# gk969/stm32-speech-recognition

Hardware: AMD Instinct MI355X
Metric: utterances/sec (256-frame, 100 templates) (higher is better)
Workload: dtype int32

## Files before the change

### include/sr_engine.h

```cpp
#ifndef SR_ENGINE_H
#define SR_ENGINE_H

#include <stddef.h>
#include <stdint.h>

#ifdef __cplusplus
extern "C" {
#endif

#define SR_OK 0
#define SR_ERR_NO_DEVICE 1
#define SR_ERR_BAD_CONFIG 2
#define SR_ERR_BAD_ARG 3
#define SR_ERR_NO_TEMPLATES 4
#define SR_ERR_HIP 5

#define SR_ST_OK 0
#define SR_ST_VAD_FAIL 1
#define SR_ST_MFCC_FAIL 2
#define SR_ST_SEG_OOB 3

#define SR_DIS_ERR 0xFFFFFFFFu
#define SR_SAVE_MASK 12345u

// ... 32 lines not shown
    uint32_t frm_num;
    uint32_t status;
} sr_result;

typedef struct sr_engine sr_engine;

void sr_default_config(sr_config *cfg);
int sr_create(const sr_config *cfg, sr_engine **out);
void sr_destroy(sr_engine *h);
const char *sr_last_error(void);

typedef struct sr_tables {
    uint16_t *hamm;
    uint16_t *tri_cen;
    uint16_t *tri_even;
    uint16_t *tri_odd;
    int8_t *dct;
    int16_t *tw_kr;
    int16_t *tw_ki;
    uint32_t *log_thr;
} sr_tables;
int sr_build_tables(const sr_config *cfg, const sr_tables *out);
int sr_build_tie_table(int8_t *out);
int sr_log_table_mismatches(void);
uint32_t sr_mag_cheap_bound(const sr_engine *h);
uint32_t sr_mag_table(uint16_t *out, uint32_t n);

int sr_set_templates(sr_engine *h, const void *store, uint32_t n_slots, uint32_t stride_bytes);
int sr_set_templates_dense(sr_engine *h, const int16_t *mfcc, const uint32_t *frames, const uint8_t *valid,
                           uint32_t n_templates, uint32_t tpl_stride);
uint32_t sr_num_templates(const sr_engine *h);
int sr_train_store(sr_engine *h, const uint16_t *pcm, uint64_t pcm_stride, uint32_t buf_len, uint32_t n,
                   const uint32_t *slot, void *store, uint32_t n_slots, uint32_t stride_bytes, uint32_t *status);

int sr_recognize_batch(sr_engine *h, const uint16_t *pcm, uint64_t pcm_stride, uint32_t buf_len, uint32_t B,
                       sr_result *results, uint32_t *scores, int16_t *mfcc, sr_vad_rec *vad);
int sr_recognize_batch_dev(sr_engine *h, const uint16_t *d_pcm, uint64_t pcm_stride, uint32_t buf_len, uint32_t B,
                           sr_result *d_results, uint32_t *d_scores, int16_t *d_mfcc, sr_vad_rec *d_vad,
                           void *stream);
int sr_recognize_batch_packed12(sr_engine *h, const uint8_t *packed, uint64_t row_stride_bytes, uint32_t buf_len, uint32_t B,
                                sr_result *results, uint32_t *scores, int16_t *mfcc, sr_vad_rec *vad);

int sr_recognize_segments_batch(sr_engine *h, const uint16_t *pcm, uint64_t pcm_stride, uint32_t buf_len, uint32_t B,
                                sr_result *results, uint32_t *scores, sr_vad_rec *vad);
int sr_recognize_segments_batch_dev(sr_engine *h, const uint16_t *d_pcm, uint64_t pcm_stride, uint32_t buf_len,
                                    uint32_t B, sr_result *d_results, uint32_t *d_scores, sr_vad_rec *d_vad,
// ... 498 lines not shown
```

### stm32_speech_recognition_amd/csrc/k_mfcc.hip

```cpp
#include "sr_fft_dev.h"

#include <type_traits>

namespace sr {

constexpr int kMfccWaves = 4;
constexpr int kFramesPerWave = 16, kFramesPerWaveMid = 4, kFramesPerWaveSmall = 1;
#ifndef SR_MAG_TAB_BINS
#define SR_MAG_TAB_BINS 8
#endif
constexpr int mfcc_tab_bins(int fpw) { return fpw == kFramesPerWave ? SR_MAG_TAB_BINS : 0; }
static_assert(SR_MAG_TAB_BINS == 0 || SR_MAG_TAB_BINS == 4 || SR_MAG_TAB_BINS == 8, "table bins per lane");
#ifndef SR_MFCC_PIPE
#define SR_MFCC_PIPE 1
#endif
#ifndef SR_MFCC_PIPE_PEEL
#define SR_MFCC_PIPE_PEEL 1
#endif
#ifndef SR_MFCC_PIPE_VMCNT
#define SR_MFCC_PIPE_VMCNT (SR_MFCC_PIPE_PEEL ? 3 : 0)
#endif
static_assert(SR_MFCC_PIPE_VMCNT == 0 || (SR_MFCC_PIPE_VMCNT == 3 && SR_MFCC_PIPE_PEEL), "younger loads counted by the wait");
constexpr bool mfcc_pipelined(int fpw) { return SR_MFCC_PIPE && mfcc_tab_bins(fpw) == 8; }
#ifndef SR_MFCC_TM_REGS
#define SR_MFCC_TM_REGS 1
#endif
#ifdef SR_INJECT_LDS_RACE
#undef SR_MFCC_TM_REGS
#define SR_MFCC_TM_REGS 0
#endif
constexpr bool mfcc_tm_regs(int fpw) { return SR_MFCC_TM_REGS && mfcc_pipelined(fpw); }
constexpr int kMelPad = kMel + 1;
__device__ __forceinline__ constexpr int mel_prefix_word(int j) { return 64 * (j & 7) + (j >> 3); }
#pragma clang diagnostic push
#pragma clang diagnostic ignored "-Winline-asm"
__device__ __forceinline__ void mel_prefix_store(uint32_t base, const uint32_t (&pe)[8], const uint32_t (&po)[8])
{
    static_assert(kBins == 512, "the offsets below are written out for two halves of 512 words");
    asm volatile("s_mov_b32 m0, %16\n\ts_nop 0\n\t"
                 "ds_write_addtid_b32 %0\n\tds_write_addtid_b32 %1 offset:256\n\tds_write_addtid_b32 %2 offset:512\n\t"
                 "ds_write_addtid_b32 %3 offset:768\n\tds_write_addtid_b32 %4 offset:1024\n\tds_write_addtid_b32 %5 offset:1280\n\t"
                 "ds_write_addtid_b32 %6 offset:1536\n\tds_write_addtid_b32 %7 offset:1792\n\t"
                 "ds_write_addtid_b32 %8 offset:2048\n\tds_write_addtid_b32 %9 offset:2304\n\tds_write_addtid_b32 %10 offset:2560\n\t"
                 "ds_write_addtid_b32 %11 offset:2816\n\tds_write_addtid_b32 %12 offset:3072\n\tds_write_addtid_b32 %13 offset:3328\n\t"
                 "ds_write_addtid_b32 %14 offset:3584\n\tds_write_addtid_b32 %15 offset:3840"
                 :
                 : "v"(pe[0]), "v"(pe[1]), "v"(pe[2]), "v"(pe[3]), "v"(pe[4]), "v"(pe[5]), "v"(pe[6]), "v"(pe[7]), "v"(po[0]),
                   "v"(po[1]), "v"(po[2]), "v"(po[3]), "v"(po[4]), "v"(po[5]), "v"(po[6]), "v"(po[7]), "s"(base)
                 : "m0", "memory");
}
__device__ __forceinline__ void mel_energy_store(uint32_t base, const uint32_t (&en)[8])
{
    static_assert(4 * energy_plane(1) == 256 && 4 * energy_plane(2) == 528 && 4 * energy_plane(3) == 784 && 4 * energy_plane(4) == 1040 &&
                      4 * energy_plane(5) == 1296 && 4 * energy_plane(6) == 1568 && 4 * energy_plane(7) == 1824 && kBins == kEnergyBins,
                  "the offsets below are written out for these plane bases");
    asm volatile("s_mov_b32 m0, %8\n\ts_nop 0\n\t"
                 "ds_write_addtid_b32 %0\n\tds_write_addtid_b32 %1 offset:256\n\tds_write_addtid_b32 %2 offset:528\n\t"
                 "ds_write_addtid_b32 %3 offset:784\n\tds_write_addtid_b32 %4 offset:1040\n\tds_write_addtid_b32 %5 offset:1296\n\t"
                 "ds_write_addtid_b32 %6 offset:1568\n\tds_write_addtid_b32 %7 offset:1824"
                 :
                 : "v"(en[0]), "v"(en[2]), "v"(en[4]), "v"(en[6]), "v"(en[1]), "v"(en[3]), "v"(en[5]), "v"(en[7]), "s"(base)
                 : "m0", "memory");
}
#pragma clang diagnostic pop
constexpr int mfcc_wave_lds_words(int fpw) { return kXchgWords + fpw * kMelPad + 64; }

template <typename Base>
struct MfccTabArgs : Base {
    const uint16_t *mag_q;
    uint32_t mag_table_off;
};
template <typename Base>
constexpr int mfcc_feat_kind<MfccTabArgs<Base>> = mfcc_feat_kind<Base>;
template <typename Base>
static MfccTabArgs<Base> mfcc_tab_args(const Base &b, const MfccMagTab &tab)
{
    MfccTabArgs<Base> r;
    static_cast<Base &>(r) = b;
    r.mag_q = tab.mag_q;
    r.mag_table_off = tab.mag_table_off;
    return r;
}

template <int kFPW, typename Args = MfccTabArgs<MfccArgs>>
__global__ void __launch_bounds__(64 * kMfccWaves, 4) k_mfcc(const Args a)
{
    constexpr int kFeat = mfcc_feat_kind<Args>;
    constexpr uint32_t kFeatW = (kFeat == SR_FEAT_FFT || kFeat == SR_FEAT_MAG) ? kBins : kMel;
    constexpr int kWaveLdsWords = mfcc_wave_lds_words(kFPW);
    constexpr int kTabBins = mfcc_tab_bins(kFPW);
    constexpr bool kPipe = mfcc_pipelined(kFPW);
    constexpr bool kTmRegs = mfcc_tm_regs(kFPW);
    extern __shared__ __attribute__((aligned(16))) uint32_t smem[];
    __shared__ uint32_t s_dctM[kCoef * kMelPad];
    __shared__ int s_dctS[kCoef * kMelPad];
    __shared__ u32x4 s_tw3[kTw3Row * 4], s_tw5[8 * 64];
    __shared__ u32x4 s_tm[4 * 64];
    const int lane = threadIdx.x & 63, w = __builtin_amdgcn_readfirstlane(threadIdx.x >> 6);
    uint32_t *buf = smem + w * kWaveLdsWords;
    uint32_t *xw = buf;
    uint32_t *powb = buf + kXchgWords, *moff = powb + kFPW * kMelPad;
    const uint32_t buf_lds = (uint32_t)(uintptr_t)(const __attribute__((address_space(3))) uint32_t *)buf;
    (void)buf_lds;

    for (int i = threadIdx.x; i < kCoef * kMel; i += blockDim.x) {
        const int c = a.t.dct[i], o = (i / kMel) * kMelPad + i % kMel;
        s_dctM[o] = (uint32_t)(((c < 0 ? -c : c) * 262144 + 99) / 100);
        s_dctS[o] = (c > 0) - (c < 0);
    }
    __syncthreads();

    LaneTw tw;
    load_lane_tw(a.t, lane, lane >> 4, tw);
    real_leg_tw(tw);
    if (w == 0 && (lane & 15) == 0) {
        const uint32_t *f = &tw.s3[0][0][0];
        const int d0 = lane >> 4;
#pragma unroll
        for (int c = 0; c < 8; c++) s_tw3[d0 * kTw3Row + c] = u32x4{f[4 * c], f[4 * c + 1], f[4 * c + 2], f[4 * c + 3]};
    }
    if (w == 1 % kMfccWaves) store_tw32(s_tw5, lane, tw.s5);
    u32x4 tm_r[4];
    if constexpr (kTmRegs) {
#pragma unroll
        for (int c = 0; c < 2; c++) {
            tm_r[c] = *(const u32x4 *)(a.t.tri_even_m + 8 * lane + 4 * c);
            tm_r[c + 2] = *(const u32x4 *)(a.t.tri_odd_m + 8 * lane + 4 * c);
        }
    }
#ifndef SR_INJECT_LDS_RACE
    if (!kTmRegs && w == 2 % kMfccWaves) {
#pragma unroll
        for (int c = 0; c < 2; c++) {
            s_tm[64 * c + lane] = *(const u32x4 *)(a.t.tri_even_m + 8 * lane + 4 * c);
            s_tm[64 * (c + 2) + lane] = *(const u32x4 *)(a.t.tri_odd_m + 8 * lane + 4 * c);
        }
    }
#endif
    __syncthreads();
#ifdef SR_INJECT_LDS_RACE
    if (w == 2 % kMfccWaves) {
#if SR_INJECT_LDS_RACE >= 2
        __builtin_amdgcn_s_sleep(127);
#endif
#pragma unroll
        for (int c = 0; c < 2; c++) {
            s_tm[64 * c + lane] = *(const u32x4 *)(a.t.tri_even_m + 8 * lane + 4 * c);
            s_tm[64 * (c + 2) + lane] = *(const u32x4 *)(a.t.tri_odd_m + 8 * lane + 4 * c);
        }
    }
#endif
    int hamm_m[3];
#pragma unroll
    for (int k = 0; k < 3; k++) hamm_m[k] = (lane + 64 * k < kFrameLen) ? hamm_fused_multiplier(a.t.hamm[lane + 64 * k]) : 0;
    int f_lo = 0, p_hi = 0, p_lo = 0, x_hi = 0, x_lo = 0;
    if (lane < kMel) {
        const int h = lane;
        f_lo = (h == 0) ? 0 : (int)a.t.tri_cen[h - 1];
        const int f_hi = (h == kMel - 1) ? kBins : (int)a.t.tri_cen[h + 1];
        const int ih = f_hi - 1, il = f_lo ? f_lo - 1 : 0, half = (h & 1) ? kBins : 0;
        p_hi = half + mel_prefix_word(ih), x_hi = (ih >> 3) > 0 ? (ih >> 3) - 1 : 0;
        p_lo = half + mel_prefix_word(il), x_lo = (il >> 3) > 0 ? (il >> 3) - 1 : 0;
    }
    const uint64_t mag_p = (uint64_t)a.mag_q;
    const u32x4 mag_rs = {(uint32_t)mag_p, (uint32_t)(mag_p >> 32) | (2u << 16), kMagTabEntries, 0x00027000u};
    const uint32_t tw_off = 32u * (uint32_t)lane;
    const int c0 = energy_read_base(lane), c1 = c0 + 4;

    uint32_t item = blockIdx.x;
    uint32_t nx_nfrm = 0;
    int nx_mid = 0, nx_seg0 = 0;
    if (item < a.n_items) {
        const sr_vad_rec *rec = a.vad + item / a.tiles;
        nx_nfrm = rec->frm_num;
        nx_mid = (int)rec->atap.mid_val;
        nx_seg0 = rec->seg[0];
    }
    for (; item < a.n_items; item += gridDim.x) {
        const uint32_t b = item / a.tiles, tile = item - b * a.tiles;
        const uint32_t nfrm = nx_nfrm;
        const int mid = nx_mid, seg0 = nx_seg0;
        if (item + gridDim.x < a.n_items) {
            const sr_vad_rec *rec = a.vad + (item + gridDim.x) / a.tiles;
            nx_nfrm = rec->frm_num;
            nx_mid = (int)rec->atap.mid_val;
            nx_seg0 = rec->seg[0];
        }
        const uint16_t *row = a.pcm + (uint64_t)b * a.pcm_stride;
        int16_t *out = a.mfcc + (uint64_t)b * a.max_frames * kCoef;
        const uint32_t f0 = tile * (kMfccWaves * kFPW) + w * kFPW;
        uint32_t *frow = nullptr;
        if constexpr (kFeat != 0) frow = a.feat + (uint64_t)b * a.max_frames * kFeatW;
        uint32_t nf = 0;
        if (f0 < nfrm) nf = (nfrm - f0 < (uint32_t)kFPW) ? nfrm - f0 : (uint32_t)kFPW;

        uint32_t s_pp[3] = {0, 0, 0};
        if (nf) {
            const uint16_t *x = row + seg0 + (int)kHop * (int)f0;
#pragma unroll
            for (int k = 0; k < 3; k++) {
                const int i = lane + 64 * k;
                if (i < kFrameLen) s_pp[k] = *(const u32_align2 *)(x + i - 1);
            }
        }
        auto store_prefixes = [&](const uint32_t (&pe)[8], const uint32_t (&po)[8]) { mel_prefix_store(buf_lds, pe, po); };
        auto store_energies = [&](const uint32_t (&en)[8]) { mel_energy_store(buf_lds, en); };
        auto exchange = [&](const uint32_t (&v)[4][4], uint32_t (&u)[4][4]) { fft_exchange_tid(buf, buf_lds, lane, v, u); };
        if constexpr (!kPipe)
        for (uint32_t fi = 0; fi < nf; fi++) {
#pragma unroll
            for (int k = 0; k < 3; k++) {
                const int i = lane + 64 * k;
                if (i < kFrameLen) k == 0 ? window_store<0>(xw, i, s_pp[k], mid, hamm_m[k]) : window_store<1>(xw, i, s_pp[k], mid, hamm_m[k]);
            }
            if (fi + 1 < nf) {
                const uint16_t *x = row + seg0 + (int)kHop * (int)(f0 + fi + 1);
#pragma unroll
// ... 358 lines not shown
            for (uint32_t t = lane; t < nf * kFeatW; t += 64) {
                const uint32_t fi = t / kFeatW, h = t - fi * kFeatW;
                fw[t] = powb[fi * kMelPad + h] >> 14;
            }
        }
        {
            int16_t *out_w = out + (size_t)f0 * kCoef;
#pragma unroll
            for (uint32_t tl = lane; tl < (uint32_t)(kFPW * kCoef); tl += 64) {
                uint32_t t = tl;
                if constexpr (kPipe) asm volatile("" : "+v"(t));
                if (t < nf * kCoef) {
                    const uint32_t fi = umul24(t, 10923u) >> 17, h = t - umul24(fi, (uint32_t)kCoef);
                    const uint32_t *pw = powb + umul24(fi, (uint32_t)kMelPad), *dm = s_dctM + umul24(h, (uint32_t)kMelPad);
                    const int *ds = s_dctS + umul24(h, (uint32_t)kMelPad);
                    int acc = 0;
#pragma unroll
                    for (int i = 0; i < kMel; i++) acc = mad24((int)__umulhi(pw[i], dm[i]), ds[i], acc);
                    out_w[t] = (int16_t)acc;
                }
            }
        }
        wave_sync();
        {
            const uint32_t r0 = f0 + nf, r1 = (f0 + kFPW < a.max_frames) ? f0 + kFPW : a.max_frames;
            for (uint32_t t = r0 * kCoef + lane; t < r1 * kCoef && r0 < r1; t += 64) out[t] = 0;
        }
        if constexpr (kFeat != 0) {
            const uint32_t r0 = f0 + nf, r1 = (f0 + kFPW < a.max_frames) ? f0 + kFPW : a.max_frames;
            for (uint32_t t = r0 * kFeatW + lane; t < r1 * kFeatW && r0 < r1; t += 64) frow[t] = 0;
        }
    }
}

uint32_t mfcc_ext_frames_per_tile();
int mfcc_ext_occupancy(int *per_cu);
void launch_mfcc_ext(const MfccArgs &a, uint32_t grid, hipStream_t s);
void launch_mfcc_ext_features(const MfccArgs &a, int kind, uint32_t *feat, uint32_t grid, hipStream_t s);

uint32_t mfcc_frames_per_tile(uint32_t frame_len) { return frame_len == 320 ? mfcc_ext_frames_per_tile() : (uint32_t)(kMfccWaves * kFramesPerWave); }
uint32_t mfcc_frames_per_tile_small(uint32_t frame_len, uint32_t which)
{
    return frame_len == 320 ? mfcc_ext_frames_per_tile() : (uint32_t)(kMfccWaves * (which ? kFramesPerWaveSmall : kFramesPerWaveMid));
}

uint32_t mfcc_resident_workgroups(uint32_t frame_len)
{
    int dev = 0, n_cu = 0, per_cu = 0;
    if (hipGetDevice(&dev) != hipSuccess) return 0;
    if (hipDeviceGetAttribute(&n_cu, hipDeviceAttributeMultiprocessorCount, dev) != hipSuccess || n_cu < 1) return 0;
    int e;
    if (frame_len == 320)
        e = mfcc_ext_occupancy(&per_cu);
    else
// ... 77 lines not shown
```

### stm32_speech_recognition_amd/csrc/sr_device.h

```cpp
#pragma once
#include <hip/hip_runtime.h>

#include <cstdint>

#include "../../include/sr_engine.h"
#include "sr_onepass_plan.h"

namespace sr {

enum DevHook {
    kHookDtwU,
    kHookDtwTieG,
    kHookDtwKc,
    kHookMfccGrid,
    kHookPerturbLogThr,
    kHookLogThrFromHost,
    kHookMultiAllowDup,
    kHookDtwDebug,
    kHookCellsLiteral,
    kHookMagCheapOff,
    kHookMagTableOff,
    kHookStreamTile,
    kHookSpotChunk,
    kHookAlignPairs,
// ... 154 lines not shown
void launch_live_scan(const LiveArgs &a, bool sad, hipStream_t s);
void launch_live_records(const LiveRecArgs &a, uint32_t n, hipStream_t s);

struct MfccArgs {
    const uint16_t *pcm;
    uint64_t pcm_stride;
    uint32_t B;
    uint32_t max_frames;
    const sr_vad_rec *vad;
    int16_t *mfcc;
    uint32_t tiles;
    uint32_t small_tiles;
    uint32_t n_items;
    uint32_t grid_cap;
    uint32_t mag_cheap_max;
    uint32_t frame_len;
    uint32_t generic;
    uint32_t hop, n_mel, n_coef;
    DevTables t;
};
struct MfccMagTab {
    const uint16_t *mag_q;
    uint32_t mag_table_off;
};

template <int kKind>
struct MfccFeatArgs : MfccArgs {
    uint32_t *feat;
};
template <typename Args>
constexpr int mfcc_feat_kind = 0;
template <int kKind>
constexpr int mfcc_feat_kind<MfccFeatArgs<kKind>> = kKind;
template <int kKind>
inline MfccFeatArgs<kKind> mfcc_feat_args(const MfccArgs &a, uint32_t *feat)
{
    MfccFeatArgs<kKind> f;
    static_cast<MfccArgs &>(f) = a;
    f.feat = feat;
    return f;
}

struct DtwArgs {
    const int16_t *mfcc;
    const sr_vad_rec *vad;
    const uint32_t *in_frames;
// ... 490 lines not shown
```

### stm32_speech_recognition_amd/csrc/sr_engine.cpp

```cpp
#include "sr_engine_internal.h"

#include <atomic>
#include <cstdio>
#include <cstdlib>

namespace sr {

static thread_local std::string g_err;
int set_error(int code, const std::string &msg)
{
    g_err = msg;
    return code;
}

#ifdef SR_TESTING
static std::atomic<int64_t> g_hooks[kHookCount];
int64_t dev_hook(DevHook h) { return g_hooks[h].load(std::memory_order_relaxed); }
static const char *const kHookNames[kHookCount] = {"dtw_u", "dtw_tie_g", "dtw_kc", "mfcc_grid", "perturb_log_thr",
                                                   "log_thr_from_host", "multi_allow_dup", "dtw_debug", "cells_literal",
                                                   "mag_cheap_off", "mag_table_off", "stream_tile_frames", "spot_chunk_cols",
                                                   "align_pairs", "align_marks_global", "chain_chunk_cols", "chain_rows", "span_groups",
                                                   "cluster_pairs", "forced_prune_off", "onepass_block", "onepass_rows", "onepass_gram_prune_off", "live_origin",
                                                   "spot_live_origin", "lds_poison_launches"};
#endif
// ... 137 lines not shown
        static bool once = false;
        if (!once) std::fprintf(stderr, "sr_engine: %s\n", msg.c_str());
        once = true;
    }
}

int sr_build_tables(const sr_config *cfg, const sr_tables *out)
{
    if (!cfg || !out) return fail(SR_ERR_BAD_ARG, "null argument");
    FrontEnd fe;
    int rc = front_end_of(cfg, &fe);
    if (rc) return rc;
    HostTables t;
    build_tables(t, fe);
    warn_log_table();
    if (out->hamm) std::memcpy(out->hamm, t.hamm.data(), t.hamm.size() * 2);
    if (out->tri_cen) std::memcpy(out->tri_cen, t.tri_cen.data(), t.tri_cen.size() * 2);
    if (out->tri_even) std::memcpy(out->tri_even, t.tri_even.data(), t.tri_even.size() * 2);
    if (out->tri_odd) std::memcpy(out->tri_odd, t.tri_odd.data(), t.tri_odd.size() * 2);
    if (out->dct) std::memcpy(out->dct, t.dct.data(), t.dct.size());
    if (out->tw_kr) std::memcpy(out->tw_kr, t.tw_kr.data(), t.tw_kr.size() * 2);
    if (out->tw_ki) std::memcpy(out->tw_ki, t.tw_ki.data(), t.tw_ki.size() * 2);
    if (out->log_thr) std::memcpy(out->log_thr, t.log_thr.data(), t.log_thr.size() * 4);
    return SR_OK;
}

int sr_build_tie_table(int8_t *out)
{
    if (!out) return fail(SR_ERR_BAD_ARG, "null argument");
    HostTables t;
    build_tables(t, kFrontRef);
    if (t.tie_delta.size() != (size_t)kTieMax) return fail(SR_ERR_BAD_CONFIG, "internal: DTW tie-threshold table does not fit 8 bits");
    std::memcpy(out, t.tie_delta.data(), t.tie_delta.size());
    return SR_OK;
}

int sr_create(const sr_config *cfg, sr_engine **out)
{
    if (!cfg || !out) return fail(SR_ERR_BAD_ARG, "null argument");
    *out = nullptr;
    FrontEnd fe;
    if (int rcf = front_end_of(cfg, &fe)) return rcf;
    if (cfg->max_frames < 2 || cfg->max_frames > 16383) return fail(SR_ERR_BAD_CONFIG, "max_frames must be 2..16383");
    if (cfg->max_seg < 1 || cfg->max_seg > SR_MAX_SEG) return fail(SR_ERR_BAD_CONFIG, "max_seg must be 1..3");
    const uint32_t noise_len = (cfg->fs / 1000) * cfg->noise_len_ms, atap_frm = (cfg->fs / 1000) * 30;
    if (noise_len == 0 || noise_len % atap_frm != 0 || noise_len % (uint32_t)fe.frame_len != 0)
// ... 46 lines not shown
            delete h;
            return fail(SR_ERR_HIP, std::string("hipFuncSetAttribute(") + kernel + ", MaxDynamicSharedMemorySize): " + hipGetErrorString(hipGetLastError()));
        }
    }
    build_tables(h->host, fe);
    warn_log_table();
    const HostTables &t = h->host;
    std::vector<uint32_t> te32(t.tri_even.begin(), t.tri_even.end()), to32(t.tri_odd.begin(), t.tri_odd.end());
    std::vector<uint32_t> tem(t.tri_even.size()), tom(t.tri_odd.size());
    for (size_t i = 0; i < tem.size(); i++) {
        if (t.tri_even[i] > kMelTriMax || t.tri_odd[i] > kMelTriMax) {
            delete h;
            return fail(SR_ERR_BAD_CONFIG, "internal: Mel triangle weight above the fused multiplier's range");
        }
        tem[i] = mel_fused_multiplier(t.tri_even[i]);
        tom[i] = mel_fused_multiplier(t.tri_odd[i]);
    }
    if (!h->generic && h->frame_len == (uint32_t)kFrameLen && (t.tri_cen.empty() || t.tri_cen[0] < 9)) {
        delete h;
        return fail(SR_ERR_BAD_CONFIG, "internal: first Mel centre below bin 9");
    }
    std::vector<uint32_t> hpk(t.hamm.size() / 2);
    for (size_t i = 0; i < hpk.size(); i++) hpk[i] = (uint32_t)t.hamm[2 * i] | ((uint32_t)t.hamm[2 * i + 1] << 16);
    struct Part {
        const void *src;
        size_t bytes;
        size_t off;
    } parts[17] = {{t.hamm.data(), t.hamm.size() * 2, 0},       {t.tri_even.data(), t.tri_even.size() * 2, 0},
                  {t.tri_odd.data(), t.tri_odd.size() * 2, 0}, {t.tri_cen.data(), t.tri_cen.size() * 2, 0},
                  {t.dct.data(), t.dct.size(), 0},             {t.tw_a.data(), t.tw_a.size() * 4, 0},
                  {t.tw_b.data(), t.tw_b.size() * 4, 0},       {t.log_thr.data(), t.log_thr.size() * 4, 0},
                  {t.w512_a.data(), t.w512_a.size() * 4, 0},   {t.w512_b.data(), t.w512_b.size() * 4, 0},
                  {te32.data(), te32.size() * 4, 0},           {to32.data(), to32.size() * 4, 0},
                  {t.tie_delta.data(), t.tie_delta.size(), 0}, {hpk.data(), hpk.size() * 4, 0},
                  {tem.data(), tem.size() * 4, 0},             {tom.data(), tom.size() * 4, 0},
                  {t.mag_q.data(), t.mag_q.size() * 2, 0}};
    if (t.tie_delta.size() != (size_t)kTieMax) {
        delete h;
        return fail(SR_ERR_BAD_CONFIG, "internal: DTW tie-threshold table does not fit 8 bits");
    }
    size_t total = 0;
    for (auto &p : parts) {
        p.off = total;
        total += (p.bytes + 255) & ~(size_t)255;
    }
    std::vector<uint8_t> blob(total, 0);
    for (auto &p : parts) std::memcpy(blob.data() + p.off, p.src, p.bytes);
    hipError_t e = hipMalloc(&h->table_blob, total);
    if (e == hipSuccess) e = hipMemcpy(h->table_blob, blob.data(), total, hipMemcpyHostToDevice);
    if (e != hipSuccess) {
        delete h;
        return fail(SR_ERR_HIP, std::string("table upload: ") + hipGetErrorString(e));
    }
    uint8_t *base = (uint8_t *)h->table_blob;
    h->dev.hamm = (const uint16_t *)(base + parts[0].off);
    h->dev.tri_even = (const uint16_t *)(base + parts[1].off);
    h->dev.tri_odd = (const uint16_t *)(base + parts[2].off);
    h->dev.tri_cen = (const uint16_t *)(base + parts[3].off);
    h->dev.dct = (const int8_t *)(base + parts[4].off);
    h->dev.tw_a = (const uint32_t *)(base + parts[5].off);
    h->dev.tw_b = (const uint32_t *)(base + parts[6].off);
    h->dev.log_thr = (const uint32_t *)(base + parts[7].off);
    h->dev.w512_a = (const uint32_t *)(base + parts[8].off);
    h->dev.w512_b = (const uint32_t *)(base + parts[9].off);
    h->dev.tri_even32 = (const uint32_t *)(base + parts[10].off);
    h->dev.tri_odd32 = (const uint32_t *)(base + parts[11].off);
    h->dev.tie_delta = (const int8_t *)(base + parts[12].off);
    h->dev.hamm_pk = (const uint32_t *)(base + parts[13].off);
    h->dev.tri_even_m = (const uint32_t *)(base + parts[14].off);
    h->dev.tri_odd_m = (const uint32_t *)(base + parts[15].off);
    h->dev_mag_q = (const uint16_t *)(base + parts[16].off);
    if (!h->generic && h->frame_len == (uint32_t)kFrameLen) {
        uint32_t *sw = nullptr;
        const uint32_t init[4] = {0, 0, 0xFFFFFFFFu, 0};
        uint32_t back[4] = {1, 0, 0, 0};
        hipError_t se = hipMalloc(&sw, sizeof init);
        if (se == hipSuccess) se = hipMemcpy(sw, init, sizeof init, hipMemcpyHostToDevice);
        if (se == hipSuccess) {
            launch_mag_fast_sweep(kMagCheapMax, (unsigned long long *)sw, sw + 2, nullptr);
            se = hipGetLastError();
        }
        if (se == hipSuccess) se = hipMemcpy(back, sw, sizeof back, hipMemcpyDeviceToHost);
        if (sw) (void)hipFree(sw);
        if (se != hipSuccess) {
            sr_destroy(h);
            return fail(SR_ERR_HIP, std::string("magnitude sweep: ") + hipGetErrorString(se));
        }
        const bool ok = back[0] == 0 && back[1] == 0;
        h->mag_cheap_max = ok ? kMagCheapMax : 0u;
        if (dev_hook(kHookMagCheapOff)) h->mag_cheap_max = 0;
        if (!ok) {
            char msg[160];
            std::snprintf(msg, sizeof msg, "sr_create: v_sqrt_f32 magnitude differs from the exact form at n = %u on this device; "
                          "every frame takes the exact root", back[2]);
// ... 321 lines not shown
```

### stm32_speech_recognition_amd/csrc/sr_engine_internal.h

```cpp
#pragma once
#include <hip/hip_runtime.h>

#include <algorithm>
#include <cstdint>
#include <cstring>
#include <string>
#include <vector>

#include "sr_device.h"
#include "sr_dtw_plan.h"
#include "sr_gram_compile.h"
#include "sr_tables.h"

namespace sr {

int set_error(int code, const std::string &msg);
static inline int fail(int code, const std::string &msg) { return set_error(code, msg); }

#define HIP_TRY(expr)                                                                                  \
    do {                                                                                               \
        hipError_t e_ = (expr);                                                                        \
        if (e_ != hipSuccess)                                                                          \
            return fail(SR_ERR_HIP, std::string(#expr) + ": " + hipGetErrorString(e_));                \
    } while (0)
// ... 45 lines not shown
    }
};

template <typename T>
struct TmpDevBuf : DevBuf<T> {
    TmpDevBuf() = default;
    TmpDevBuf(const TmpDevBuf &) = delete;
    ~TmpDevBuf() { this->release(); }
};

}

using namespace sr;

static constexpr uint32_t kVadWideBelow = 1024, kMfccFill = 1024;
static constexpr uint32_t kPairCounters = 65536;

struct sr_engine {
    sr_config cfg;
    int device = 0;
    uint32_t noise_len = 0, atap_frm = 0;
    uint32_t n_cu = 256;
    LdsBudget lds;
    const uint16_t *dev_mag_q = nullptr;
    uint32_t mag_cheap_max = 0;
    uint32_t mfcc_tile = 64, mfcc_tile_mid = 64, mfcc_tile_small = 64, mfcc_grid_cap = 0;
    uint32_t frame_len = 160, hop = 80;
    uint32_t nc = 12, n_mel = 24;
    size_t mfcc_elems(size_t B) const { return B * cfg.max_frames * nc; }
    bool generic = false;
    uint32_t v_durmin = 8, s_durmax = 11;
    HostTables host;
    DevTables dev{};
    void *table_blob = nullptr;
    DevBuf<int16_t> tpl;
    DevBuf<uint32_t> tpl_frames;
    DevBuf<uint8_t> tpl_valid;
    bool tpl_staged_ok = true;
    DevBuf<uint32_t> tplR;
    DevBuf<uint32_t> tpl_frames_s, tpl_orig;
    DevBuf<uint32_t> tpl_rank;
    uint32_t K = 0, tpl_rows = 0, tpl_stride = 0;
    uint64_t store_serial = 0;
    DtwPlan plan;
    uint32_t dp_lanes = 0;
    std::vector<uint32_t> cells_by_len;
// ... 148 lines not shown
```

### stm32_speech_recognition_amd/csrc/sr_fft_dev.h

```cpp
#pragma once
#include <type_traits>

#include "sr_dev.h"
#include "sr_fft_layout.h"

namespace sr {

__device__ __forceinline__ void cxmul(uint32_t y, uint32_t ka, uint32_t kb, int &re, int &im)
{
    re = sdot2z(y, ka);
    im = sdot2z(y, kb);
}

template <int S>
__device__ __forceinline__ void r4_combine(int &ar, int &ai, int &br, int &bi, int &cr, int &ci, int &dr, int &di)
{
    int tr = cr + dr, ti = ci + di;
    dr = cr - dr;
    di = ci - di;
    cr = tr;
    ci = ti;
    ar >>= 2;
    ai >>= 2;
    ar += br >> (2 + S);
// ... 173 lines not shown
    load_tw4(t, 60, lane, tw.s4);
#pragma unroll
    for (int d3 = 0; d3 < 4; d3++) load_tw4(t, 252, lane + 64 * d3, tw.s5[d3]);
}

__device__ __forceinline__ void store_tw32(u32x4 *lds, int lane, const uint32_t (&k)[4][4][2])
{
    const uint32_t *f = &k[0][0][0];
#pragma unroll
    for (int c = 0; c < 8; c++) lds[c * 64 + lane] = u32x4{f[4 * c], f[4 * c + 1], f[4 * c + 2], f[4 * c + 3]};
}
__device__ __forceinline__ void load_tw32(const u32x4 *lds, int lane, uint32_t (&k)[4][4][2])
{
    uint32_t *f = &k[0][0][0];
#pragma unroll
    for (int c = 0; c < 8; c++) {
        const u32x4 q = lds[c * 64 + lane];
        f[4 * c] = q.x;
        f[4 * c + 1] = q.y;
        f[4 * c + 2] = q.z;
        f[4 * c + 3] = q.w;
    }
}
constexpr int kTw3Row = 9;
__device__ __forceinline__ void load_tw32_d0(const u32x4 *lds, int d0, uint32_t (&k)[4][4][2])
{
    uint32_t *f = &k[0][0][0];
#pragma unroll
    for (int c = 0; c < 8; c++) {
        const u32x4 q = lds[d0 * kTw3Row + c];
        f[4 * c] = q.x;
        f[4 * c + 1] = q.y;
        f[4 * c + 2] = q.z;
        f[4 * c + 3] = q.w;
    }
}

constexpr uint32_t kPkOneTwo = 0x00020001u;
template <int K>
__device__ __forceinline__ void window_store(uint32_t *xw, int i, uint32_t prev_cur, int mid, int hm)
{
    if (K == 0) {
        xw[i] = pk_mul_lo_dup(window_sample<4>(prev_cur, mid, hm), kPkOneTwo);
    } else {
        const uint32_t y = window_sample<2>(prev_cur, mid, hm);
        xw[i] = y;
        ((uint16_t *)(xw + i))[1] = (uint16_t)y;
// ... 158 lines not shown
```

### stm32_speech_recognition_amd/csrc/sr_launch.cpp

```cpp
#include "sr_engine_internal.h"

using namespace sr;
int check_batch(const sr_engine *h, uint32_t B)
{
    const uint32_t tile = std::min(h->mfcc_tile, std::min(h->mfcc_tile_mid, h->mfcc_tile_small));
    if ((uint64_t)B * ((h->cfg.max_frames + tile - 1) / tile) > 0xFFFFFFFFull) return fail(SR_ERR_BAD_ARG, "batch too large");
    return SR_OK;
}

int mark_scratch_user(sr_engine *h, hipStream_t s)
{
    if (!h->ev_scratch) HIP_TRY(hipEventCreateWithFlags(&h->ev_scratch, hipEventDisableTiming));
    HIP_TRY(hipEventRecord(h->ev_scratch, s));
    h->scratch_pending = true;
    return SR_OK;
}
int order_after_scratch_users(sr_engine *h, hipStream_t s)
{
    if (!h->scratch_pending) return SR_OK;
    if (hipEventQuery(h->ev_scratch) == hipSuccess) {
        h->scratch_pending = false;
        return SR_OK;
    }
    (void)hipGetLastError();
// ... 47 lines not shown
    if (h->mfcc_tile_small < h->mfcc_tile && h->small_launch != 1) {
        const uint32_t t_mid = (h->cfg.max_frames + h->mfcc_tile_mid - 1) / h->mfcc_tile_mid;
        const uint32_t t_small = (h->cfg.max_frames + h->mfcc_tile_small - 1) / h->mfcc_tile_small;
        if (h->small_launch == 2 || (uint64_t)B * t_mid < kMfccFill) {
            a.tiles = t_small;
            a.small_tiles = 2;
        } else if ((uint64_t)B * a.tiles < kMfccFill) {
            a.tiles = t_mid;
            a.small_tiles = 1;
        }
    }
    a.grid_cap = h->mfcc_grid_cap;
    a.mag_cheap_max = h->mag_cheap_max;
    a.frame_len = h->frame_len;
    a.n_items = B * a.tiles;
    a.generic = h->generic ? 1u : 0u;
    a.hop = h->hop;
    a.n_mel = h->n_mel;
    a.n_coef = h->nc;
    a.t = h->dev;
    return a;
}

MfccMagTab mfcc_mag_tab(const sr_engine *h) { return MfccMagTab{h->dev_mag_q, dev_hook(kHookMagTableOff) ? 1u : 0u}; }

int sr_mfcc_batch_dev(sr_engine *h, const uint16_t *d_pcm, uint64_t pcm_stride, uint32_t B, const sr_vad_rec *d_vad,
                      int16_t *d_mfcc, void *stream)
{
    if (!h || !d_pcm || !d_vad || !d_mfcc) return fail(SR_ERR_BAD_ARG, "null argument");
    if (pcm_stride >= (1ull << 31)) return fail(SR_ERR_BAD_ARG, "pcm_stride must be below 2^31 samples");
    if (int rcb = check_batch(h, B)) return rcb;
    ENTER_DEVICE(h);
    launch_mfcc(mfcc_args(h, d_pcm, pcm_stride, B, d_vad, d_mfcc), mfcc_mag_tab(h), (hipStream_t)stream);
    HIP_TRY(hipGetLastError());
    return SR_OK;
}

DtwArgs dtw_args(const sr_engine *h, const int16_t *d_mfcc, const sr_vad_rec *d_vad, const uint32_t *d_in_frames,
                        uint32_t B, uint32_t *d_scores, sr_result *d_results)
{
    DtwArgs a;
    a.mfcc = d_mfcc;
    a.vad = d_vad;
    a.in_frames = d_in_frames;
    a.B = B;
    a.max_frames = h->cfg.max_frames;
    a.tpl = h->tpl.p;
// ... 313 lines not shown
```

### stm32_speech_recognition_amd/csrc/sr_tables.cpp

```cpp
#include "sr_device.h"
#include "sr_tables.h"

#include <atomic>
#include <cmath>
#include <cstdio>
#include <cstdlib>

namespace sr {

static const uint32_t kLogThrRef[kLogMax + 2] = {
#include "sr_log_thr_ref.inc"
};
static std::atomic<int> g_log_mismatches{0};
int log_table_mismatches() { return g_log_mismatches.load(); }

static double mround(double v) { return v >= 0.0 ? std::floor(v + 0.5) : -std::floor(-v + 0.5); }

static void gen_hamm(HostTables &t, const FrontEnd &fe)
{
    t.hamm.resize(fe.frame_len);
    for (int i = 0; i < fe.frame_len; i++)
        t.hamm[i] = (uint16_t)mround((0.54 - 0.46 * std::cos(2 * M_PI * i / (fe.frame_len - 1))) * 10000.0);
}

// ... 111 lines not shown
}

static uint32_t root_u32(uint32_t d) { return (uint32_t)sqrtf((float)d); }

static void gen_tie_delta(HostTables &t)
{
    t.tie_delta.assign(kTieMax, 1);
    for (uint32_t g = 4095; g < (uint32_t)kTieMax; g++) {
        const uint64_t M = (uint64_t)(g + 1) * (g + 1);
        uint32_t d = (uint32_t)M;
        while (root_u32(d - 1) >= g + 1) d--;
        const int64_t delta = (int64_t)d - (int64_t)M + 1;
        t.tie_delta[g] = (int8_t)delta;
        if (delta < -128 || delta > 127) t.tie_delta.clear();
    }
}

void gen_mag_q(std::vector<uint16_t> &out)
{
    out.resize(kMagTabEntries);
    for (uint32_t n = 0; n < kMagTabEntries; n++) out[n] = (uint16_t)(((uint32_t)(sqrtf((float)n) * 10.0f)) << 2);
}

void build_tables(HostTables &t, const FrontEnd &fe)
{
    gen_mag_q(t.mag_q);
    gen_tie_delta(t);
    gen_hamm(t, fe);
    gen_tri(t, fe);
    gen_dct(t, fe);
    gen_twiddles(t);
    gen_log_thr(t);
    gen_w512(t);
}

}
```

### stm32_speech_recognition_amd/csrc/sr_tables.h

```cpp
#pragma once
#include <cstdint>
#include <vector>

namespace sr {

constexpr int kFrameLen = 160;
constexpr int kHop = 80;
constexpr int kNfft = 1024;
constexpr int kBins = 512;
constexpr int kMel = 24;
constexpr int kCoef = 12;
constexpr int kTwiddles = 1020;
constexpr int kLogMax = 2218;
constexpr int kTieMax = 32768;


constexpr int kWinShift = 5;
constexpr int32_t hamm_fused_multiplier(uint32_t h) { return (int32_t)((((uint64_t)h << 27) + 999u) / 1000u); }

constexpr uint32_t kMelFusedMaxE = (1u << 28) / 100u;
constexpr uint32_t kMagSmallMax = 26843;
static_assert(1638u * 1638u <= kMelFusedMaxE && 100ull * (kMagSmallMax + 1) < 1639ull * 1639ull, "quiet-frame bound");
constexpr uint32_t kMagCheapMax = 70171;
static_assert(kMagSmallMax <= kMagCheapMax, "the quiet tier lies inside the cheap-magnitude range");
// ... 3 lines not shown
constexpr uint32_t mel_fused_multiplier(uint32_t tri) { return (uint32_t)((((uint64_t)tri << 28) + 99u) / 100u); }

struct FrontEnd {
    int fs, frame_len, hop, nfft, bins, n_mel, n_coef;
    bool generic;
};
constexpr FrontEnd kFrontRef = {8000, 160, 80, 1024, 512, 24, 12, false};
constexpr FrontEnd kFrontExt = {16000, 320, 160, 512, 256, 40, 12, false};

struct HostTables {
    std::vector<uint16_t> hamm;
    std::vector<uint16_t> tri_cen;
    std::vector<uint16_t> tri_even;
    std::vector<uint16_t> tri_odd;
    std::vector<int8_t> dct;
    std::vector<uint32_t> tw_a, tw_b;
    std::vector<int16_t> tw_kr, tw_ki;
    std::vector<uint32_t> log_thr;
    std::vector<uint32_t> w512_a, w512_b;
    std::vector<int8_t> tie_delta;
    std::vector<uint16_t> mag_q;
};

void build_tables(HostTables &t, const FrontEnd &fe);
void gen_mag_q(std::vector<uint16_t> &out);
int log_table_mismatches();

}
```

### stm32_speech_recognition_amd/engine.py

```python
import ctypes as C
import os

import numpy as np

_HERE = os.path.dirname(os.path.abspath(__file__))
LIB_PATH = os.path.join(_HERE, "libsr_engine.so")
TESTING_LIB_PATH = os.path.join(_HERE, "libsr_engine_testing.so")

DIS_ERR = 0xFFFFFFFF
ST_OK, ST_VAD_FAIL, ST_MFCC_FAIL, ST_SEG_OOB = 0, 1, 2, 3
N_COEF = 12
FEAT_FFT, FEAT_MAG, FEAT_MEL, FEAT_LOGMEL = 1, 2, 3, 4

RESULT_DTYPE = np.dtype([("best_tpl", "<u4"), ("min_dis", "<u4"), ("frm_num", "<u4"), ("status", "<u4")])
VAD_DTYPE = np.dtype([("mid_val", "<u4"), ("n_thl", "<u2"), ("z_thl", "<u2"), ("s_thl", "<u4"),
                      ("seg", "<i4", (6,)), ("frm_num", "<u4"), ("status", "<u4"), ("_pad", "<u4")])
ATAP_DTYPE = np.dtype([("mid_val", "<u4"), ("n_thl", "<u2"), ("z_thl", "<u2"), ("s_thl", "<u4")])
STREAM_SEG_DTYPE = np.dtype([("stream", "<u4"), ("start", "<i4"), ("end", "<i4"), ("frm_num", "<u4")])
NBEST_DTYPE = np.dtype([("word", "<u4"), ("slot", "<u4"), ("dis", "<u4"), ("count", "<u4")])
NO_WORD, NBEST_MAX = 0xFFFFFFFF, 16
LIVE_SEG_DTYPE = np.dtype([("channel", "<u4"), ("frm_num", "<u4"), ("start", "<i8"), ("end", "<i8")])
SPOT_DTYPE = np.dtype([("dis", "<u4"), ("start", "<u4"), ("end", "<u4"), ("acc", "<u4")])
SPOT_WIN_DTYPE = np.dtype([("channel", "<u4"), ("window", "<u4")])
ALIGN_DTYPE = np.dtype([("dis", "<u4"), ("acc", "<u4"), ("path_len", "<u4"), ("status", "<u4")])
# ... 83 lines not shown
    _fields_ = [(n, C.c_void_p) for n in ("hamm", "tri_cen", "tri_even", "tri_odd", "dct", "tw_kr", "tw_ki", "log_thr")]


def build_tables(**kw):
    L = load_library()
    cfg = Config()
    L.sr_default_config(C.byref(cfg))
    for k, v in kw.items():
        setattr(cfg, k, v)
    frame_len, nb = cfg.fs // 1000 * cfg.frame_time_ms, cfg.nfft // 2
    out = dict(hamm=np.zeros(frame_len, np.uint16), tri_cen=np.zeros(cfg.n_mel, np.uint16),
               tri_even=np.zeros(nb, np.uint16), tri_odd=np.zeros(nb, np.uint16),
               dct=np.zeros(cfg.n_coef * cfg.n_mel, np.int8), tw_kr=np.zeros(1020, np.int16),
               tw_ki=np.zeros(1020, np.int16), log_thr=np.zeros(2220, np.uint32))
    t = _Tables(**{k: v.ctypes.data_as(C.c_void_p) for k, v in out.items()})
    rc = L.sr_build_tables(C.byref(cfg), C.byref(t))
    if rc != 0:
        raise SrError(f"sr_build_tables error {rc}: {L.sr_last_error().decode()}")
    out["tie_delta"] = np.zeros(32768, np.int8)
    rc = L.sr_build_tie_table(out["tie_delta"].ctypes.data_as(C.c_void_p))
    if rc != 0:
        raise SrError(f"sr_build_tie_table error {rc}: {L.sr_last_error().decode()}")
    return out


class Engine:

    def __init__(self, max_frames=119, device=-1, testing=False, **kw):
        self.L = load_library(testing)
        self._testing, self._kw, self._tpl = testing, dict(kw), None
        cfg = Config()
        self.L.sr_default_config(C.byref(cfg))
        cfg.max_frames = max_frames
        cfg.device = device
        for k, v in kw.items():
            setattr(cfg, k, v)
        self.cfg = cfg
        h = C.c_void_p()
        self._check(self.L.sr_create(C.byref(cfg), C.byref(h)))
        self.h = h
        self.max_frames = max_frames
        self.n_coef = cfg.n_coef
        self.noise_len = (cfg.fs // 1000) * cfg.noise_len_ms

    @classmethod
    def borrowed(cls, handle, cfg, max_frames, lib=None):
# ... 1813 lines not shown
```

Before: 3.508 million.

## Precompute MFCC per-lane constants on host and bulk-load into LDS

After: 3.524 million (median of 6 runs). Within noise of the previous version (+0.4%).

```diff
diff --git a/include/sr_engine.h b/include/sr_engine.h
--- a/include/sr_engine.h
+++ b/include/sr_engine.h
@@ -78,6 +78,7 @@
 } sr_tables;
 int sr_build_tables(const sr_config *cfg, const sr_tables *out);
 int sr_build_tie_table(int8_t *out);
+int sr_build_mfcc_const(uint32_t *out, uint32_t cap_words, uint32_t *n_words);
 int sr_log_table_mismatches(void);
 uint32_t sr_mag_cheap_bound(const sr_engine *h);
 uint32_t sr_mag_table(uint16_t *out, uint32_t n);
diff --git a/stm32_speech_recognition_amd/csrc/k_mfcc.hip b/stm32_speech_recognition_amd/csrc/k_mfcc.hip
--- a/stm32_speech_recognition_amd/csrc/k_mfcc.hip
+++ b/stm32_speech_recognition_amd/csrc/k_mfcc.hip
@@ -30,8 +30,6 @@
 #define SR_MFCC_TM_REGS 0
 #endif
 constexpr bool mfcc_tm_regs(int fpw) { return SR_MFCC_TM_REGS && mfcc_pipelined(fpw); }
-constexpr int kMelPad = kMel + 1;
-__device__ __forceinline__ constexpr int mel_prefix_word(int j) { return 64 * (j & 7) + (j >> 3); }
 #pragma clang diagnostic push
 #pragma clang diagnostic ignored "-Winline-asm"
 __device__ __forceinline__ void mel_prefix_store(uint32_t base, const uint32_t (&pe)[8], const uint32_t (&po)[8])
@@ -69,6 +67,7 @@
 struct MfccTabArgs : Base {
     const uint16_t *mag_q;
     uint32_t mag_table_off;
+    const uint32_t *lane_const;
 };
 template <typename Base>
 constexpr int mfcc_feat_kind<MfccTabArgs<Base>> = mfcc_feat_kind<Base>;
@@ -79,6 +78,7 @@
     static_cast<Base &>(r) = b;
     r.mag_q = tab.mag_q;
     r.mag_table_off = tab.mag_table_off;
+    r.lane_const = tab.lane_const;
     return r;
 }
 
@@ -91,11 +91,17 @@
     constexpr int kTabBins = mfcc_tab_bins(kFPW);
     constexpr bool kPipe = mfcc_pipelined(kFPW);
     constexpr bool kTmRegs = mfcc_tm_regs(kFPW);
+    constexpr bool kConst = kFPW == kFramesPerWave;
     extern __shared__ __attribute__((aligned(16))) uint32_t smem[];
-    __shared__ uint32_t s_dctM[kCoef * kMelPad];
-    __shared__ int s_dctS[kCoef * kMelPad];
-    __shared__ u32x4 s_tw3[kTw3Row * 4], s_tw5[8 * 64];
-    __shared__ u32x4 s_tm[4 * 64];
+    __shared__ u32x4 s_const[kMfccConstShared];
+    uint32_t *const s_dctM = (uint32_t *)(s_const + kMfccConstDctM);
+    int *const s_dctS = (int *)(s_const + kMfccConstDctS);
+    u32x4 *const s_tw3 = s_const + kMfccConstTw3, *const s_tw5 = s_const + kMfccConstTw5;
+    u32x4 *s_tm = nullptr;
+    if constexpr (!kTmRegs) {
+        __shared__ u32x4 s_tm_lds[4 * 64];
+        s_tm = s_tm_lds;
+    }
     const int lane = threadIdx.x & 63, w = __builtin_amdgcn_readfirstlane(threadIdx.x >> 6);
     uint32_t *buf = smem + w * kWaveLdsWords;
     uint32_t *xw = buf;
@@ -103,23 +109,48 @@
     const uint32_t buf_lds = (uint32_t)(uintptr_t)(const __attribute__((address_space(3))) uint32_t *)buf;
     (void)buf_lds;
 
-    for (int i = threadIdx.x; i < kCoef * kMel; i += blockDim.x) {
-        const int c = a.t.dct[i], o = (i / kMel) * kMelPad + i % kMel;
-        s_dctM[o] = (uint32_t)(((c < 0 ? -c : c) * 262144 + 99) / 100);
-        s_dctS[o] = (c > 0) - (c < 0);
-    }
-    __syncthreads();
-
     LaneTw tw;
-    load_lane_tw(a.t, lane, lane >> 4, tw);
-    real_leg_tw(tw);
-    if (w == 0 && (lane & 15) == 0) {
-        const uint32_t *f = &tw.s3[0][0][0];
-        const int d0 = lane >> 4;
-#pragma unroll
-        for (int c = 0; c < 8; c++) s_tw3[d0 * kTw3Row + c] = u32x4{f[4 * c], f[4 * c + 1], f[4 * c + 2], f[4 * c + 3]};
-    }
-    if (w == 1 % kMfccWaves) store_tw32(s_tw5, lane, tw.s5);
+    int hamm_m[3];
+    int f_lo = 0, p_hi = 0, p_lo = 0, x_hi = 0, x_lo = 0;
+    if constexpr (kConst) {
+        const u32x4 *cb = (const u32x4 *)a.lane_const;
+        constexpr int kThreads = 64 * kMfccWaves, kRounds = (kMfccConstShared + kThreads - 1) / kThreads;
+        u32x4 sc[kRounds];
+#pragma unroll
+        for (int r = 0; r < kRounds; r++) {
+            const int i = (int)threadIdx.x + r * kThreads;
+            if ((r + 1) * kThreads <= kMfccConstShared || i < kMfccConstShared) sc[r] = cb[i];
+        }
+        const u32x4 *lc = cb + kMfccConstLane + lane;
+        const u32x4 q0 = lc[0], q1 = lc[64], q2 = lc[128], q3 = lc[192], q4 = lc[256];
+#pragma unroll
+        for (int r = 0; r < kRounds; r++) {
+            const int i = (int)threadIdx.x + r * kThreads;
+            if ((r + 1) * kThreads <= kMfccConstShared || i < kMfccConstShared) s_const[i] = sc[r];
+        }
+        hamm_m[0] = (int)q0.x, hamm_m[1] = (int)q0.y, hamm_m[2] = (int)q0.z, f_lo = (int)q0.w;
+        p_hi = (int)q1.x, p_lo = (int)q1.y, x_hi = (int)q1.z, x_lo = (int)q1.w;
+        tw.s2[0][0] = q2.x, tw.s2[0][1] = q2.y, tw.s2[1][0] = q2.z, tw.s2[1][1] = q2.w;
+        tw.s4[0][0] = q3.x, tw.s4[0][1] = q3.y, tw.s4[1][0] = q3.z, tw.s4[1][1] = q3.w;
+        tw.s4[2][0] = q4.x, tw.s4[2][1] = q4.y, tw.s4[3][0] = q4.z, tw.s4[3][1] = q4.w;
+    } else {
+        for (int i = threadIdx.x; i < kCoef * kMel; i += blockDim.x) {
+            const int c = a.t.dct[i], o = (i / kMel) * kMelPad + i % kMel;
+            s_dctM[o] = (uint32_t)(((c < 0 ? -c : c) * 262144 + 99) / 100);
+            s_dctS[o] = (c > 0) - (c < 0);
+        }
+        __syncthreads();
+
+        load_lane_tw(a.t, lane, lane >> 4, tw);
+        real_leg_tw(tw);
+        if (w == 0 && (lane & 15) == 0) {
+            const uint32_t *f = &tw.s3[0][0][0];
+            const int d0 = lane >> 4;
+#pragma unroll
+            for (int c = 0; c < 8; c++) s_tw3[d0 * kTw3Row + c] = u32x4{f[4 * c], f[4 * c + 1], f[4 * c + 2], f[4 * c + 3]};
+        }
+        if (w == 1 % kMfccWaves) store_tw32(s_tw5, lane, tw.s5);
+    }
     u32x4 tm_r[4];
     if constexpr (kTmRegs) {
 #pragma unroll
@@ -150,17 +181,17 @@
         }
     }
 #endif
-    int hamm_m[3];
-#pragma unroll
-    for (int k = 0; k < 3; k++) hamm_m[k] = (lane + 64 * k < kFrameLen) ? hamm_fused_multiplier(a.t.hamm[lane + 64 * k]) : 0;
-    int f_lo = 0, p_hi = 0, p_lo = 0, x_hi = 0, x_lo = 0;
-    if (lane < kMel) {
-        const int h = lane;
-        f_lo = (h == 0) ? 0 : (int)a.t.tri_cen[h - 1];
-        const int f_hi = (h == kMel - 1) ? kBins : (int)a.t.tri_cen[h + 1];
-        const int ih = f_hi - 1, il = f_lo ? f_lo - 1 : 0, half = (h & 1) ? kBins : 0;
-        p_hi = half + mel_prefix_word(ih), x_hi = (ih >> 3) > 0 ? (ih >> 3) - 1 : 0;
-        p_lo = half + mel_prefix_word(il), x_lo = (il >> 3) > 0 ? (il >> 3) - 1 : 0;
+    if constexpr (!kConst) {
+#pragma unroll
+        for (int k = 0; k < 3; k++) hamm_m[k] = (lane + 64 * k < kFrameLen) ? hamm_fused_multiplier(a.t.hamm[lane + 64 * k]) : 0;
+        if (lane < kMel) {
+            const int h = lane;
+            f_lo = (h == 0) ? 0 : (int)a.t.tri_cen[h - 1];
+            const int f_hi = (h == kMel - 1) ? kBins : (int)a.t.tri_cen[h + 1];
+            const int ih = f_hi - 1, il = f_lo ? f_lo - 1 : 0, half = (h & 1) ? kBins : 0;
+            p_hi = half + mel_prefix_word(ih), x_hi = (ih >> 3) > 0 ? (ih >> 3) - 1 : 0;
+            p_lo = half + mel_prefix_word(il), x_lo = (il >> 3) > 0 ? (il >> 3) - 1 : 0;
+        }
     }
     const uint64_t mag_p = (uint64_t)a.mag_q;
     const u32x4 mag_rs = {(uint32_t)mag_p, (uint32_t)(mag_p >> 32) | (2u << 16), kMagTabEntries, 0x00027000u};
@@ -193,6 +224,22 @@
         if constexpr (kFeat != 0) frow = a.feat + (uint64_t)b * a.max_frames * kFeatW;
         uint32_t nf = 0;
         if (f0 < nfrm) nf = (nfrm - f0 < (uint32_t)kFPW) ? nfrm - f0 : (uint32_t)kFPW;
+        auto zero_rows = [&]() {
+            const uint32_t r0 = f0 + nf, r1 = (f0 + kFPW < a.max_frames) ? f0 + kFPW : a.max_frames;
+            const uint32_t n = r0 < r1 ? (r1 - r0) * kCoef : 0u;
+            int16_t *z = out + (size_t)r0 * kCoef;
+#pragma unroll
+            for (uint32_t t = lane; t < (uint32_t)(kFPW * kCoef); t += 64)
+                if (t < n) z[t] = 0;
+            if constexpr (kFeat != 0)
+                for (uint32_t t = r0 * kFeatW + lane; t < r1 * kFeatW && r0 < r1; t += 64) frow[t] = 0;
+        };
+        if constexpr (kConst) {
+            if (nf == 0) {
+                zero_rows();
+                continue;
+            }
+        }
 
         uint32_t s_pp[3] = {0, 0, 0};
         if (nf) {
@@ -597,14 +644,7 @@
             }
         }
         wave_sync();
-        {
-            const uint32_t r0 = f0 + nf, r1 = (f0 + kFPW < a.max_frames) ? f0 + kFPW : a.max_frames;
-            for (uint32_t t = r0 * kCoef + lane; t < r1 * kCoef && r0 < r1; t += 64) out[t] = 0;
-        }
-        if constexpr (kFeat != 0) {
-            const uint32_t r0 = f0 + nf, r1 = (f0 + kFPW < a.max_frames) ? f0 + kFPW : a.max_frames;
-            for (uint32_t t = r0 * kFeatW + lane; t < r1 * kFeatW && r0 < r1; t += 64) frow[t] = 0;
-        }
+        zero_rows();
     }
 }
 
diff --git a/stm32_speech_recognition_amd/csrc/sr_device.h b/stm32_speech_recognition_amd/csrc/sr_device.h
--- a/stm32_speech_recognition_amd/csrc/sr_device.h
+++ b/stm32_speech_recognition_amd/csrc/sr_device.h
@@ -200,6 +200,7 @@
 struct MfccMagTab {
     const uint16_t *mag_q;
     uint32_t mag_table_off;
+    const uint32_t *lane_const;
 };
 
 template <int kKind>
diff --git a/stm32_speech_recognition_amd/csrc/sr_engine.cpp b/stm32_speech_recognition_amd/csrc/sr_engine.cpp
--- a/stm32_speech_recognition_amd/csrc/sr_engine.cpp
+++ b/stm32_speech_recognition_amd/csrc/sr_engine.cpp
@@ -183,6 +183,18 @@
     if (out->tw_kr) std::memcpy(out->tw_kr, t.tw_kr.data(), t.tw_kr.size() * 2);
     if (out->tw_ki) std::memcpy(out->tw_ki, t.tw_ki.data(), t.tw_ki.size() * 2);
     if (out->log_thr) std::memcpy(out->log_thr, t.log_thr.data(), t.log_thr.size() * 4);
+    return SR_OK;
+}
+
+int sr_build_mfcc_const(uint32_t *out, uint32_t cap_words, uint32_t *n_words)
+{
+    HostTables t;
+    build_tables(t, kFrontRef);
+    std::vector<uint32_t> c;
+    build_mfcc_const(t, c);
+    if (!out || cap_words < c.size()) return fail(SR_ERR_BAD_ARG, "null argument or fewer than " + std::to_string(c.size()) + " words");
+    std::memcpy(out, c.data(), c.size() * 4);
+    if (n_words) *n_words = (uint32_t)c.size();
     return SR_OK;
 }
 
@@ -275,11 +287,13 @@
     }
     std::vector<uint32_t> hpk(t.hamm.size() / 2);
     for (size_t i = 0; i < hpk.size(); i++) hpk[i] = (uint32_t)t.hamm[2 * i] | ((uint32_t)t.hamm[2 * i + 1] << 16);
+    std::vector<uint32_t> mconst;
+    if (!h->generic && h->frame_len == (uint32_t)kFrameLen) build_mfcc_const(t, mconst);
     struct Part {
         const void *src;
         size_t bytes;
         size_t off;
-    } parts[17] = {{t.hamm.data(), t.hamm.size() * 2, 0},       {t.tri_even.data(), t.tri_even.size() * 2, 0},
+    } parts[18] = {{t.hamm.data(), t.hamm.size() * 2, 0},       {t.tri_even.data(), t.tri_even.size() * 2, 0},
                   {t.tri_odd.data(), t.tri_odd.size() * 2, 0}, {t.tri_cen.data(), t.tri_cen.size() * 2, 0},
                   {t.dct.data(), t.dct.size(), 0},             {t.tw_a.data(), t.tw_a.size() * 4, 0},
                   {t.tw_b.data(), t.tw_b.size() * 4, 0},       {t.log_thr.data(), t.log_thr.size() * 4, 0},
@@ -287,7 +301,7 @@
                   {te32.data(), te32.size() * 4, 0},           {to32.data(), to32.size() * 4, 0},
                   {t.tie_delta.data(), t.tie_delta.size(), 0}, {hpk.data(), hpk.size() * 4, 0},
                   {tem.data(), tem.size() * 4, 0},             {tom.data(), tom.size() * 4, 0},
-                  {t.mag_q.data(), t.mag_q.size() * 2, 0}};
+                  {t.mag_q.data(), t.mag_q.size() * 2, 0},     {mconst.data(), mconst.size() * 4, 0}};
     if (t.tie_delta.size() != (size_t)kTieMax) {
         delete h;
         return fail(SR_ERR_BAD_CONFIG, "internal: DTW tie-threshold table does not fit 8 bits");
@@ -323,6 +337,7 @@
     h->dev.tri_even_m = (const uint32_t *)(base + parts[14].off);
     h->dev.tri_odd_m = (const uint32_t *)(base + parts[15].off);
     h->dev_mag_q = (const uint16_t *)(base + parts[16].off);
+    h->dev_mfcc_const = mconst.empty() ? nullptr : (const uint32_t *)(base + parts[17].off);
     if (!h->generic && h->frame_len == (uint32_t)kFrameLen) {
         uint32_t *sw = nullptr;
         const uint32_t init[4] = {0, 0, 0xFFFFFFFFu, 0};
diff --git a/stm32_speech_recognition_amd/csrc/sr_engine_internal.h b/stm32_speech_recognition_amd/csrc/sr_engine_internal.h
--- a/stm32_speech_recognition_amd/csrc/sr_engine_internal.h
+++ b/stm32_speech_recognition_amd/csrc/sr_engine_internal.h
@@ -91,6 +91,7 @@
     uint32_t noise_len = 0, atap_frm = 0;
     uint32_t n_cu = 256;
     LdsBudget lds;
+    const uint32_t *dev_mfcc_const = nullptr;
     const uint16_t *dev_mag_q = nullptr;
     uint32_t mag_cheap_max = 0;
     uint32_t mfcc_tile = 64, mfcc_tile_mid = 64, mfcc_tile_small = 64, mfcc_grid_cap = 0;
diff --git a/stm32_speech_recognition_amd/csrc/sr_fft_dev.h b/stm32_speech_recognition_amd/csrc/sr_fft_dev.h
--- a/stm32_speech_recognition_amd/csrc/sr_fft_dev.h
+++ b/stm32_speech_recognition_amd/csrc/sr_fft_dev.h
@@ -219,7 +219,6 @@
         f[4 * c + 3] = q.w;
     }
 }
-constexpr int kTw3Row = 9;
 __device__ __forceinline__ void load_tw32_d0(const u32x4 *lds, int d0, uint32_t (&k)[4][4][2])
 {
     uint32_t *f = &k[0][0][0];
diff --git a/stm32_speech_recognition_amd/csrc/sr_launch.cpp b/stm32_speech_recognition_amd/csrc/sr_launch.cpp
--- a/stm32_speech_recognition_amd/csrc/sr_launch.cpp
+++ b/stm32_speech_recognition_amd/csrc/sr_launch.cpp
@@ -93,7 +93,7 @@
     return a;
 }
 
-MfccMagTab mfcc_mag_tab(const sr_engine *h) { return MfccMagTab{h->dev_mag_q, dev_hook(kHookMagTableOff) ? 1u : 0u}; }
+MfccMagTab mfcc_mag_tab(const sr_engine *h) { return MfccMagTab{h->dev_mag_q, dev_hook(kHookMagTableOff) ? 1u : 0u, h->dev_mfcc_const}; }
 
 int sr_mfcc_batch_dev(sr_engine *h, const uint16_t *d_pcm, uint64_t pcm_stride, uint32_t B, const sr_vad_rec *d_vad,
                       int16_t *d_mfcc, void *stream)
diff --git a/stm32_speech_recognition_amd/csrc/sr_tables.cpp b/stm32_speech_recognition_amd/csrc/sr_tables.cpp
--- a/stm32_speech_recognition_amd/csrc/sr_tables.cpp
+++ b/stm32_speech_recognition_amd/csrc/sr_tables.cpp
@@ -157,6 +157,54 @@
     for (uint32_t n = 0; n < kMagTabEntries; n++) out[n] = (uint16_t)(((uint32_t)(sqrtf((float)n) * 10.0f)) << 2);
 }
 
+void build_mfcc_const(const HostTables &t, std::vector<uint32_t> &out)
+{
+    out.assign((size_t)kMfccConstChunks * 4, 0u);
+    for (int i = 0; i < kCoef * kMel; i++) {
+        const int c = t.dct[i], o = (i / kMel) * kMelPad + i % kMel;
+        out[4 * kMfccConstDctM + o] = (uint32_t)(((c < 0 ? -c : c) * 262144 + 99) / 100);
+        out[4 * kMfccConstDctS + o] = (uint32_t)((c > 0) - (c < 0));
+    }
+    auto neg_pk = [](uint32_t v) { return ((0u - (v & 0xFFFFu)) & 0xFFFFu) | ((0u - (v >> 16)) << 16); };
+    auto tw4 = [&](int base, int b, uint32_t *k) {
+        const int e = base + 3 * b;
+        for (int leg = 0; leg < 3; leg++) {
+            k[2 * leg] = t.tw_a[e + 2 - leg];
+            k[2 * leg + 1] = t.tw_b[e + 2 - leg];
+        }
+        k[6] = neg_pk(k[4]);
+        k[7] = neg_pk(k[5]);
+    };
+    for (int d0 = 0; d0 < 4; d0++)
+        for (int d1 = 0; d1 < 4; d1++) tw4(12, d0 + 4 * d1, &out[4 * (kMfccConstTw3 + d0 * kTw3Row) + 8 * d1]);
+    for (int lane = 0; lane < 64; lane++) {
+        uint32_t f[32];
+        for (int d3 = 0; d3 < 4; d3++) tw4(252, lane + 64 * d3, f + 8 * d3);
+        for (int c = 0; c < 8; c++)
+            for (int j = 0; j < 4; j++) out[4 * (kMfccConstTw5 + 64 * c + lane) + j] = f[4 * c + j];
+        uint32_t *l0 = &out[4 * (kMfccConstLane + lane)], *l1 = l0 + 4 * 64, *l2 = l1 + 4 * 64, *l3 = l2 + 4 * 64;
+        for (int k = 0; k < 3; k++) l0[k] = (lane + 64 * k < kFrameLen) ? (uint32_t)hamm_fused_multiplier(t.hamm[lane + 64 * k]) : 0u;
+        if (lane < kMel) {
+            const int h = lane, f_lo = (h == 0) ? 0 : (int)t.tri_cen[h - 1], f_hi = (h == kMel - 1) ? kBins : (int)t.tri_cen[h + 1];
+            const int ih = f_hi - 1, il = f_lo ? f_lo - 1 : 0, half = (h & 1) ? kBins : 0;
+            l0[3] = (uint32_t)f_lo;
+            l1[0] = (uint32_t)(half + mel_prefix_word(ih));
+            l1[1] = (uint32_t)(half + mel_prefix_word(il));
+            l1[2] = (uint32_t)((ih >> 3) > 0 ? (ih >> 3) - 1 : 0);
+            l1[3] = (uint32_t)((il >> 3) > 0 ? (il >> 3) - 1 : 0);
+        }
+        uint32_t k2[8];
+        tw4(0, lane >> 4, k2);
+        for (int j = 0; j < 4; j++) l2[j] = (k2[j] & 0xFFFFu) * 0x10001u;
+        uint32_t k4[8];
+        tw4(60, lane, k4);
+        for (int j = 0; j < 4; j++) {
+            l3[j] = k4[j];
+            l3[4 * 64 + j] = k4[4 + j];
+        }
+    }
+}
+
 void build_tables(HostTables &t, const FrontEnd &fe)
 {
     gen_mag_q(t.mag_q);
diff --git a/stm32_speech_recognition_amd/csrc/sr_tables.h b/stm32_speech_recognition_amd/csrc/sr_tables.h
--- a/stm32_speech_recognition_amd/csrc/sr_tables.h
+++ b/stm32_speech_recognition_amd/csrc/sr_tables.h
@@ -49,6 +49,15 @@
     std::vector<uint16_t> mag_q;
 };
 
+constexpr int kMelPad = kMel + 1;
+constexpr int kTw3Row = 9;
+constexpr int kMfccConstDctM = 0, kMfccConstDctS = kMfccConstDctM + kCoef * kMelPad / 4, kMfccConstTw3 = kMfccConstDctS + kCoef * kMelPad / 4,
+              kMfccConstTw5 = kMfccConstTw3 + 4 * kTw3Row, kMfccConstShared = kMfccConstTw5 + 8 * 64, kMfccConstLane = kMfccConstShared,
+              kMfccConstLaneChunks = 5, kMfccConstChunks = kMfccConstLane + kMfccConstLaneChunks * 64;
+static_assert(kCoef * kMelPad % 4 == 0, "the DCT tables are whole 16-byte chunks");
+constexpr int mel_prefix_word(int j) { return 64 * (j & 7) + (j >> 3); }
+void build_mfcc_const(const HostTables &t, std::vector<uint32_t> &out);
+
 void build_tables(HostTables &t, const FrontEnd &fe);
 void gen_mag_q(std::vector<uint16_t> &out);
 int log_table_mismatches();
diff --git a/stm32_speech_recognition_amd/engine.py b/stm32_speech_recognition_amd/engine.py
--- a/stm32_speech_recognition_amd/engine.py
+++ b/stm32_speech_recognition_amd/engine.py
@@ -129,6 +129,15 @@
     if rc != 0:
         raise SrError(f"sr_build_tie_table error {rc}: {L.sr_last_error().decode()}")
     return out
+
+
+def build_mfcc_const():
+    L = load_library()
+    out, n = np.zeros(8192, np.uint32), C.c_uint32(0)
+    rc = L.sr_build_mfcc_const(out.ctypes.data_as(C.c_void_p), C.c_uint32(out.size), C.byref(n))
+    if rc != 0:
+        raise SrError(f"sr_build_mfcc_const error {rc}: {L.sr_last_error().decode()}")
+    return out[:n.value].copy()
 
 
 class Engine:
```
